# ctu-vras/monoforce

Hardware: AMD Instinct MI355X
Metric: rollout-steps/sec (batch x horizon) on 256x256 terrain (higher is better)
Workload: dtype f32; 1 GPU; c3: B=1024/GPU x T=500 x N=4 contact points, 256x256 grid (res 0.05 m), one shared terrain+friction map (the same on every rank), integrator=odeint-euler (reference default), forward+backward; BASE...; rollouts_per_gpu=1024, rollouts_total=1024, horizon=500, contact_points=4, parallelism=rollout-sharded x1

## Files before the change

monoforce_amd/csrc/rollout_bwd_cp_kernel.h:

```cpp
#pragma once
#include "rollout_bwd_kernel.h"
#include "rollout_cp_common.h"
#include "stream_ring.h"
#include <type_traits>

namespace mf {

#ifdef MF_STREAM_PROFILE
extern __device__ unsigned long long mf_stream_prof[32];
#define MF_PROF_T(v) const unsigned long long v = __builtin_readcyclecounter()
#define MF_PROF_RT(v) const unsigned long long v = __builtin_amdgcn_s_memrealtime()
#define MF_PROF_ACC(name) unsigned long long name = 0
#define MF_PROF_SUM(name, t0) name += __builtin_readcyclecounter() - (t0)
#define MF_PROF_OUT(slot, val) do { if (lane == 0) atomicAdd(&mf_stream_prof[slot], (unsigned long long)(val)); } while (0)
#define MF_PROF_ADD(slot, t0) MF_PROF_OUT(slot, __builtin_readcyclecounter() - (t0))
#define MF_PROF_MAX(slot, val) do { if (lane == 0) atomicMax(&mf_stream_prof[slot], (unsigned long long)(val)); } while (0)
#define MF_PROF_DRAIN() asm volatile("s_waitcnt vmcnt(0) lgkmcnt(0)" ::: "memory")
#else
#define MF_PROF_T(v)
#define MF_PROF_RT(v)
#define MF_PROF_ACC(name)
#define MF_PROF_SUM(name, t0)
#define MF_PROF_OUT(slot, val)
#define MF_PROF_ADD(slot, t0)
// ... 448 lines not shown
      k.wa = mf_fma(wa_s, dpp<kB0>(fr), wa_o); k.wb = mf_fma(wb_s, dpp<kB1>(fr), wb_o);
      k.wq = k.wa * k.wb;
      k.cj = v.q.y; k.wraw = v.q.z; k.A = v.q.w;
      k.idx = v.idx; k.zc = v.zc; k.mcv = has_mu ? v.mc : one;
      k.mub = dot4(k.wq, k.mcv);
      const S dz = v.zc - dpp<kB0>(v.zc);
      const S u = mf_fma(dpp<kN12>(dz), n_mul, n_add);
      k.inl = M::inv_len(dot3(u, u));
      k.nrm = u * k.inl;
      k.inv_csum = M::div(one, sum_points(k.cj));
      k.coln2 = dot3(st.R0, st.R0);
      k.il = M::inv_len(k.coln2);
      k.e = st.R0 * k.il;
      k.tv = cp_track(tv_v, tv_w, st.cv, st.cw);
      k.F0 = -(k.A * k.nrm);
      k.F1 = cp_spring(k.A, k.nrm, k.cj, k.inv_csum);
      k.Fr = M::clamp(k.F1, -mg, mg);
      k.Nn = M::sqrt(dot3(k.Fr, k.Fr));
      k.cmdv = cp_cmd(k.tv, k.e, k.vp);
      k.s = k.mub * k.cmdv;
      k.sn = dot3(k.s, k.nrm);
      k.stv = cp_tangent(k.s, k.sn, k.nrm);
      k.Gf = k.Nn * k.stv;
      const S f = k.Fr + M::clamp(k.Gf, -mg, mg);
      k.f1 = dpp<kRot1>(f); k.f2 = dpp<kRot2>(f);
    };
    const bool loss_on = STREAM && a.loss_gt != nullptr;
    const Msk loss_mask = loss_on ? ~(Msk)0 : (Msk)0;
    const S loss_scale = loss_on ? S(2.0) * a.loss_gloss[0] * a.loss_inv_count : zero;
    const S* const loss_gt_lane = loss_on ? a.loss_gt + ((size_t)b * (size_t)a.loss_T2) * 3u + (unsigned)cc : a.z;
    const int* const l_row_stamp = loss_on ? a.loss_row_stamp : reinterpret_cast<const int*>(a.ts);
    const S* const l_row_w = loss_on ? a.loss_row_w : a.ts;
    const int l_T2m1 = loss_on ? a.loss_T2 - 1 : 0;
    if constexpr (STREAM) {
      const unsigned un = (unsigned)max(n, 0);
      unsigned o3 = v3 + un * s3, o9 = v9 + un * s9, oc = v_ctrl + un * kC, orc = un * rec_step;
      constexpr unsigned kUp = ODE ? 1u : 0u;
      unsigned og_xs = u_xs + (un + kUp) * sg_xs, og_xds = u_xds + (un + kUp) * sg_xds, og_om = u_om + (un + kUp) * sg_om;
      unsigned og_r = u_r + (un + kUp) * sg_r, og_fs = u_fs + (un + kUp) * sg_fs, og_ff = u_ff + (un + kUp) * sg_ff;
      int ti = max(n, 0);
      auto request_state = [&](StateIn& d, Saved& v) {
        d.x = zero;
#ifdef MF_STREAM_NO_FETCH
        d.xd = S(0.1); d.w = S(0.01); d.R0 = cc == 0 ? one : zero; d.R1 = cc == 1 ? one : zero; d.R2 = cc == 2 ? one : zero; d.cv = S(0.5); d.cw = S(0.1);
        d.t1 = S(0.01); d.t0 = zero; v.q = f4v{S(100.3), S(0.2), S(0.1), S(50.0)};
        return;
#endif
        if constexpr (ODE) {
          d.xd = bload1<S>(rXds, o3, 0u); d.w = bload1<S>(rOm, o3, 0u);
          bload3(rRs, o9, 0u, &d.R0, &d.R1, &d.R2);
          d.t1 = a.ts[ti + 1]; d.t0 = a.ts[ti];
        } else {
          const bool init = ti == 0;
          const unsigned p3 = init ? o3 : o3 - s3, p9 = init ? o9 : o9 - s9;
          const S xd = bload1<S>(rXds, p3, 0u), w = bload1<S>(rOm, p3, 0u);
          S R0, R1, R2;
          bload3(rRs, p9, 0u, &R0, &R1, &R2);
          d.xd = init ? ini.xd : xd; d.w = init ? ini.w : w;
          d.R0 = init ? ini.R0 : R0; d.R1 = init ? ini.R1 : R1; d.R2 = init ? ini.R2 : R2;
          d.x = bload1<S>(rOm, o3, 0u);
          d.t1 = a.dt; d.t0 = zero;
        }
        bload2(rCtrl, oc, 0u, &d.cv, &d.cw);
        v.q = __builtin_nontemporal_load(reinterpret_cast<const f4v*>(prec + (size_t)orc));
      };
      auto request_up = [&](UpIn& u) {
#ifdef MF_STREAM_NO_FETCH
        u.gXs = S(0.001);
        if constexpr (!XS_ONLY) { u.gXds = u.gOm = u.gR0 = u.gR1 = u.gR2 = u.gFs = u.gFf = S(0.001); }
        return;
#endif
        u.gXs = bload1<S>(rgXs, og_xs, 0u);
        if constexpr (!XS_ONLY) {
          u.gXds = bload1<S>(rgXds, og_xds, 0u); u.gOm = bload1<S>(rgOm, og_om, 0u);
          bload3(rgRs, og_r, 0u, &u.gR0, &u.gR1, &u.gR2);
          u.gFs = bload1<S>(rgFs, og_fs, 0u); u.gFf = bload1<S>(rgFf, og_ff, 0u);
        }
      };
      auto step_back_up = [&]() {
        og_xs -= sg_xs;
        if constexpr (!XS_ONLY) { og_xds -= sg_xds; og_om -= sg_om; og_r -= sg_r; og_fs -= sg_fs; og_ff -= sg_ff; }
      };
      constexpr int kSlots = SLOTS, kPlanesD = ODE ? 0 : 6, kPlanes = (XS_ONLY ? 10 : 12) + kPlanesD;
      constexpr bool kPow2 = (kSlots & (kSlots - 1)) == 0;
      __shared__ f4v ring[kSlots * kPlanes * 64];
      __shared__ int flags[4];
      typedef __attribute__((address_space(3))) volatile int LdsCounter;
      LdsCounter* vflags = (LdsCounter*)flags;
      if (threadIdx.x == 0) { flags[0] = 0; flags[1] = 0; flags[2] = 0; flags[3] = 0; }
      constexpr unsigned kAnsPlane = 0u, kIdxPlane = 7u * 64u;
      typedef S f2v __attribute__((ext_vector_type(2)));
      if constexpr (HANDOFF) {
        for (unsigned sl = threadIdx.x >> 6; sl < (unsigned)kSlots; sl += 3u) {
          f4v* o = ring + sl * (unsigned)(kPlanes * 64) + lane;
          o[kAnsPlane] = f4v{zero, zero, zero, zero}; o[kIdxPlane] = f4v{zero, zero, zero, idx_as(zero, 0)};
        }
      }
      __syncthreads();
      const bool loss_val = loss_on && a.loss_out != nullptr;
      __shared__ S l_part[3 * 16];
      auto loss_share = [&](S acc) {
        if (!loss_val) return;
        const int wv = (int)(threadIdx.x >> 6);
        if (lane < 16) l_part[wv * 16 + lane] = zero;
        if (p == 0 && q < 3) l_part[wv * 16 + (lane >> 4) * 4 + q] = acc;
        asm volatile("" ::: "memory");
        if (lane == 0) __hip_atomic_fetch_add(&flags[2], 1, __ATOMIC_RELAXED, __HIP_MEMORY_SCOPE_WORKGROUP);
      };
      auto loss_value_finish = [&]() {
        if (!loss_val) return;
        while (__builtin_amdgcn_readfirstlane(vflags[2]) != 3) __builtin_amdgcn_s_sleep(1);
        asm volatile("" ::: "memory");
        unsigned last_wg = 0u;
        if (lane == 0) {
          S tot = zero;
#pragma unroll
          for (int r = 0; r < 4; ++r)
#pragma unroll
            for (int v = 0; v < 3; ++v) tot += (l_part[v * 16 + r * 4 + 0] + l_part[v * 16 + r * 4 + 1]) + l_part[v * 16 + r * 4 + 2];
          __builtin_nontemporal_store(tot, a.loss_partial + blockIdx.x);
          __threadfence();
          last_wg = atomicAdd(a.loss_ticket, 1u) == gridDim.x - 1 ? 1u : 0u;
        }
        last_wg = __builtin_amdgcn_readfirstlane(last_wg);
        if (last_wg) {
          __threadfence();
          const int n_act = min(64, (a.B - (int)blockIdx.x * 4) * 16);
          S tot = zero;
          for (unsigned k0 = (unsigned)lane; k0 < gridDim.x; k0 += 8u * (unsigned)n_act) {
            S v[8];
#pragma unroll
            for (int i = 0; i < 8; ++i) {
              const unsigned k2 = k0 + (unsigned)(i * n_act);
              v[i] = __builtin_nontemporal_load(a.loss_partial + min(k2, gridDim.x - 1u));
              v[i] = k2 < gridDim.x ? v[i] : zero;
            }
#pragma unroll
            for (int i = 0; i < 8; ++i) tot += v[i];
          }
          S sum = zero;
#pragma unroll
          for (int k2 = 0; k2 < 64; ++k2) sum += k2 < n_act ? mf_readlane(tot, k2) : zero;
          if (lane == 0) {
            a.loss_out[0] = sum * a.loss_inv_count;
            *a.loss_ticket = 0u;
          }
        }
      };
      __shared__ S snap_c[4 * 64];
      auto snap_prepare = [&]() {
        if (!a.skip_snap) {
          S wq, dx, dy;
          int idx;
          snap_cell(idx, wq, dx, dy);
          snap_c[lane] = idx_as(zero, idx); snap_c[64 + lane] = wq; snap_c[128 + lane] = dx; snap_c[192 + lane] = dy;
        }
        asm volatile("" ::: "memory");
        vflags[3] = 1;
      };
      if (threadIdx.x >= 64) {
        static_assert(kSlots % BATCH == 0 && (BATCH == 2 || BATCH == 3), "a batch must not wrap around the ring");
        static_assert(!HANDOFF || stream_ring::fixed_ownership(kSlots, BATCH), "hand-off: a wave reads back the answers of the steps it wrote");
        struct Slot { StateIn st; Saved sv; UpIn up; S lg, lw; int sj; };
        unsigned zero_lane = 0u;
        asm("" : "+v"(zero_lane));
        const int fk = __builtin_amdgcn_readfirstlane((int)(threadIdx.x >> 6)) - 1;
        int m = n;
        S l_acc = zero;
        auto fetch = [&](Slot& r) {
          request_state(r.st, r.sv);
          request_up(r.up);
          r.sj = ld32(l_row_stamp, (unsigned)ti + kUp + zero_lane);
          r.lw = ld32(l_row_w, (unsigned)ti + kUp + zero_lane);
          r.lg = zero;
          o3 -= s3; o9 -= s9; oc -= kC; orc -= rec_step; --ti;
          step_back_up();
          --m;
        };
        constexpr unsigned kB = (unsigned)BATCH;
        auto skip3 = [&]() {
          o3 -= kB * s3; o9 -= kB * s9; oc -= kB * kC; orc -= kB * rec_step; ti -= BATCH; m -= BATCH;
          og_xs -= kB * sg_xs;
          if constexpr (!XS_ONLY) { og_xds -= kB * sg_xds; og_om -= kB * sg_om; og_r -= kB * sg_r; og_fs -= kB * sg_fs; og_ff -= kB * sg_ff; }
        };
        MF_PROF_T(t_fetcher);
        MF_PROF_ACC(acc_room); MF_PROF_ACC(acc_pub);
        auto room = [&](int upto) {
          MF_PROF_T(t0);
          while (!stream_ring::has_room(upto - 1, __builtin_amdgcn_readfirstlane(vflags[1]), kSlots)) __builtin_amdgcn_s_sleep(2);
          asm volatile("" ::: "memory");
          MF_PROF_SUM(acc_room, t0);
        };
        int pub = 0;
        auto publish_written = [&](int upto) {
          asm volatile("" ::: "memory");
          if (__builtin_amdgcn_readfirstlane(vflags[0]) == pub) { vflags[0] = upto; pub = upto; }
        };
        auto publish = [&](int upto) {
          asm volatile("" ::: "memory");
          MF_PROF_T(t0);
          if (pub != upto) {
            while (__builtin_amdgcn_readfirstlane(vflags[0]) != pub) __builtin_amdgcn_s_sleep(1);
            asm volatile("" ::: "memory");
            vflags[0] = upto; pub = upto;
          }
          MF_PROF_SUM(acc_pub, t0);
        };
        [[maybe_unused]] auto absorb = [&](unsigned ni, S nz, S nm) {
          const bool same = !act | (ni == acc_idx);
          if (!same) emit(acc_idx, acc_z, acc_m);
          acc_idx = act ? ni : acc_idx;
          acc_z = same ? acc_z + nz : nz;
          acc_m = same ? acc_m + nm : nm;
        };
        [[maybe_unused]] auto absorb_slot = [&](unsigned slot) {
          const f4v* in = ring + slot * (unsigned)(kPlanes * 64) + lane;
          const f2v ans = *reinterpret_cast<const f2v*>(in + kAnsPlane);
          const S ib = reinterpret_cast<const S*>(in + kIdxPlane)[3];
          absorb((unsigned)idx_of(ib), ans.x, ans.y);
        };
        [[maybe_unused]] unsigned pend_idx = 0u;
        [[maybe_unused]] S pend_z = zero, pend_m = zero;
        auto put = [&](const Slot& r, unsigned slot, int o) {
            Rec k;
            rebuild(r.st, r.sv, k);
            if constexpr (HANDOFF) {
              asm("" : "+v"(pend_z), "+v"(pend_m) : "v"(k.zc), "v"(k.mcv), "v"(k.R2), "v"(k.cj), "v"(r.lg), "v"(r.up.gXs));
              absorb(pend_idx, pend_z, pend_m);
            }
            const S mw = inside(k.wraw, -a.omega_max, a.omega_max) ? one : zero;
            const S mG = inside(k.Gf, -mg, mg) ? one : zero;
            const S mF1 = inside(k.F1, -mg, mg) ? one : zero;
            const S invNn = k.Nn > zero ? M::div(one, k.Nn) : zero;
            const S cmask = k.coln2 >= S(1e-12) ? one : zero;
            const S cs = k.cj * k.inv_csum;
            const f4v p0 = f4v{k.R0, k.R1, k.R2, k.h};
            const f4v p1 = f4v{k.w1, k.w2, k.r1, k.r2};
            const f4v p2 = f4v{k.f1, k.f2, mw, mG * k.stv};
            const f4v p3 = f4v{mG * k.Nn, k.nrm, k.s, k.sn};
            const f4v p4 = f4v{k.cmdv, k.mub, k.tv * k.mub, k.Fr * invNn};
            const f4v p5 = f4v{mF1 * cs, mF1 * k.nrm, k.A, -(a.k * cs)};
            const f4v p6 = f4v{-(a.damp * cs), -(k.A * k.inv_csum), k.A * k.cj * k.inv_csum * k.inv_csum, -S(10.0) * k.cj * (one - k.cj)};
            const f4v p7 = f4v{k.vp, -(k.inl * a.inv_res), k.wq, idx_as(zero, k.idx)};
            const f4v p8 = f4v{k.zc, k.mcv, wa_s * k.wb * a.inv_res, wb_s * k.wa * a.inv_res};
            const Msk smask = r.sj >= 0 ? ~(Msk)0 : (Msk)0;
            const S gXs_row = bfi(loss_mask, bfi(smask, cp_loss_grad(loss_scale, r.up.gXs, r.lg, r.lw), zero), r.up.gXs);
            l_acc += bfi(smask, cp_loss_term(r.up.gXs, r.lg, r.lw), zero);
            const f4v p9 = f4v{k.e, k.il, cmask * k.e * k.il, first * gXs_row};
            f4v d0 = {zero, zero, zero, zero}, d1 = d0, d2 = d0, d3 = d0, d4 = d0, d5 = d0;
            if constexpr (!ODE) {
              const S h = a.dt, wn = r.st.x;
              const S th2 = dot3(wn, wn);
              const S idn = M::inv_len(th2);
              const S kv = wn * idn;
              const S th = M::sqrt(th2);
              S sn_, oc;
              M::sincos_small(th * h, &sn_, &oc);
              const S kk = dot3(kv, kv);
              const S kv1 = dpp<kRot1>(kv), kv2 = dpp<kRot2>(kv);
              const S ok = oc * kv;
              const S m0 = mf_fma(ok, kv, mf_fma(-oc, kk, one)), m1 = mf_fma(ok, kv1, -(sn_ * kv2)), m2 = mf_fma(ok, kv2, sn_ * kv1);
              const S q0 = dpp<kB0>(kv), q1 = dpp<kB1>(kv), q2 = dpp<kB2>(kv);
              const S Rk = k.R0 * q0 + k.R1 * q1 + k.R2 * q2;
              const S idn2 = th2 >= S(1e-12) ? idn * idn : zero;
              const S ith = th2 > zero ? M::div(one, th) : zero;
              d0 = f4v{wn, kv, q0, q1};
              d1 = f4v{q2, Rk, kk, sn_};
              d2 = f4v{oc, h * (one - oc), h * sn_, idn};
              d3 = f4v{idn2, ith, dpp<kB0>(m0), dpp<kB0>(m1)};
              d4 = f4v{dpp<kB0>(m2), dpp<kB1>(m2), dpp<kB1>(m0), dpp<kB1>(m1)};
              d5 = f4v{dpp<kB2>(m1), dpp<kB2>(m2), dpp<kB2>(m0), zero};
            }
            room(o + 1);
            f4v* out = ring + slot * (unsigned)(kPlanes * 64) + lane;
            [[maybe_unused]] f2v old_ans = {zero, zero};
            [[maybe_unused]] S old_idx = zero;
            if constexpr (HANDOFF) {
              old_ans = *reinterpret_cast<const f2v*>(out + kAnsPlane);
              old_idx = reinterpret_cast<const S*>(out + kIdxPlane)[3];
              asm volatile("" ::: "memory");
            }
            out[0] = p0; out[64] = p1; out[128] = p2; out[192] = p3; out[256] = p4; out[320] = p5; out[384] = p6; out[448] = p7; out[512] = p8; out[576] = p9;
            if constexpr (!XS_ONLY) {
              out[640] = f4v{first * r.up.gXds, first * r.up.gOm, r.up.gFs, r.up.gFf};
              out[704] = f4v{first * r.up.gR0, first * r.up.gR1, first * r.up.gR2, zero};
            }
            if constexpr (!ODE) {
              constexpr int D0 = (XS_ONLY ? 10 : 12) * 64;
              out[D0] = d0; out[D0 + 64] = d1; out[D0 + 128] = d2; out[D0 + 192] = d3; out[D0 + 256] = d4; out[D0 + 320] = d5;
            }
            publish_written(o + 1);
            if constexpr (HANDOFF) { pend_idx = (unsigned)idx_of(old_idx); pend_z = old_ans.x; pend_m = old_ans.y; }
#ifdef MF_STREAM_PROFILE
            if (o == 0) MF_PROF_ADD(18, t_k0);
#endif
          };
        int ord = BATCH * fk;
        unsigned sbase = kB * (unsigned)fk;
        auto fetch3 = [&](Slot (&s)[BATCH]) {
#pragma unroll
          for (int i = 0; i < BATCH; ++i) fetch(s[i]);
          skip3();
        };
        auto gather1 = [&](Slot& r) {
          gather_cells(r.sv);
          r.lg = loss_gt_lane[(size_t)(unsigned)min(max(r.sj, 0), l_T2m1) * 3u];
        };
        auto gather3 = [&](Slot (&s)[BATCH]) {
#pragma unroll
          for (int i = 0; i < BATCH; ++i) gather1(s[i]);
        };
        auto put3 = [&](const Slot (&s)[BATCH]) {
          pub = ord;
#pragma unroll
          for (int i = 0; i < BATCH; ++i) put(s[i], sbase + (unsigned)i, ord + i);
          publish(ord + BATCH);
          ord += 2 * BATCH;
          if constexpr (kSlots != 2 * BATCH) sbase = sbase + 2u * kB >= (unsigned)kSlots ? sbase + 2u * kB - (unsigned)kSlots : sbase + 2u * kB;
        };
        Slot A[BATCH], B[BATCH], C[BATCH];
        const int n_full = (n + 1) / BATCH;
        int full = (n_full - fk + 1) / 2;
        if (fk == 1) skip3();
        if (full >= 2) {
          fetch3(A); fetch3(B); gather3(A);
          full -= 2;
          while (full >= 3) {
            fetch3(C); gather3(B); put3(A);
            fetch3(A); gather3(C); put3(B);
            fetch3(B); gather3(A); put3(C);
            full -= 3;
          }
          if (full == 0) { gather3(B); put3(A); put3(B); }
          else if (full == 1) { fetch3(C); gather3(B); put3(A); gather3(C); put3(B); put3(C); }
          else { fetch3(C); gather3(B); put3(A); fetch3(A); gather3(C); put3(B); gather3(A); put3(C); put3(A); }
        } else if (full == 1) { fetch3(A); gather3(A); put3(A); }
        if (fk == (n_full & 1)) {
          int o = BATCH * n_full;
          unsigned sl = sbase;
          while (m >= 0) {
            Slot r0;
            fetch(r0);
            gather1(r0);
            pub = o;
            put(r0, sl, o);
            publish(o + 1);
            ++sl; ++o;
          }
        }
        MF_PROF_ADD(2 + 4 * fk, t_fetcher);
        MF_PROF_OUT(0 + 4 * fk, acc_room); MF_PROF_OUT(1 + 4 * fk, acc_pub);
        loss_share(l_acc);
        if (fk == 0) {
          MF_PROF_T(t_lf);
          loss_value_finish();
          MF_PROF_DRAIN();
          MF_PROF_ADD(21, t_lf);
#ifdef MF_STREAM_PROFILE
          MF_PROF_MAX(17, __builtin_readcyclecounter() - t_lf);
          MF_PROF_MAX(14, __builtin_amdgcn_s_memrealtime());
#endif
        } else {
          snap_prepare();
        }
        if constexpr (HANDOFF) {
          MF_PROF_T(t_dr);
          while (__builtin_amdgcn_readfirstlane(vflags[1]) != n_steps) __builtin_amdgcn_s_sleep(1);
          asm volatile("" ::: "memory");
          MF_PROF_ADD(25 + fk, t_dr);
          absorb(pend_idx, pend_z, pend_m);
          for (int o = stream_ring::first_undrained(n_steps, kSlots); o < n_steps; ++o)
            if (stream_ring::owner_of(o, BATCH) == fk) absorb_slot((unsigned)stream_ring::slot_of(o, kSlots));
          if (act) emit(acc_idx, acc_z, acc_m);
        }
        return;
      }
        int consumed = 0, seen = 0;
        unsigned rslot = 0u;
        UpIn uZ;
        load_upstream(0, uZ);
        S l_row0 = zero;
        if (loss_on && ODE) {
          const S g0 = loss_gt_lane[(size_t)max(a.loss_row_stamp[0], 0) * 3u], w0 = a.loss_row_w[0];
          const bool stamped = a.loss_row_stamp[0] >= 0;
          l_row0 = stamped ? cp_loss_term(uZ.gXs, g0, w0) : zero;
          uZ.gXs = stamped ? cp_loss_grad(loss_scale, uZ.gXs, g0, w0) : zero;
        }
        loss_share(l_row0);
        struct Coef {
          S R0, R1, R2, h, w1, w2, r1, r2, f1, f2, mw;
          S stvG, NnG, nrm, s, sn;
          S cmdv, mub, tvm, FrN;
          S csm, nm1, A, kcs;
          S dcs, Aic, Acc, dcj;
          S vp, inlr, wq, zc, mcv, wsb, wsa;
          S e, il, eci;
          int idx;
          unsigned off;
          S wn, kv, q0, q1, q2, Rk, kk, sn_, oc, cga, cgb, idn, idn2, ith;
          S M00, M01, M02, M10, M11, M12, M20, M21, M22;
        };
        MF_PROF_T(t_compute);
        MF_PROF_ACC(acc_wait);
#ifdef MF_STREAM_PROFILE
        unsigned long long acc_wait_early = 0, acc_wait_late = 0, n_waited = 0;
#endif
        auto ensure = [&](int k) {
          MF_PROF_T(t0);
          int have = __builtin_amdgcn_readfirstlane(seen);
          while (have < consumed + k) have = __builtin_amdgcn_readfirstlane(vflags[0]);
          asm volatile("" ::: "memory");
          MF_PROF_SUM(acc_wait, t0);
#ifdef MF_STREAM_PROFILE
          const unsigned long long dt = __builtin_readcyclecounter() - t0;
          if (consumed < 30) acc_wait_early += dt;
          if (consumed >= n_steps - 30) acc_wait_late += dt;
          n_waited += __builtin_amdgcn_readfirstlane(seen) < consumed + k ? 1u : 0u;
#endif
        };
        auto grab = [&](Coef& c, UpIn& up) {
          c.off = (kPow2 ? (unsigned)(consumed & (kSlots - 1)) : rslot) * (unsigned)(kPlanes * 64) + (unsigned)lane;
          const f4v* o = ring + c.off;
          if constexpr (!kPow2) rslot = rslot + 1u == (unsigned)kSlots ? 0u : rslot + 1u;
          const f4v c0 = o[0], c1 = o[64], c2 = o[128], c3 = o[192], c4 = o[256], c5 = o[320], c6 = o[384], c7 = o[448], c8 = o[512], c9 = o[576];
          const S idx_bits = c7.w;
          c.R0 = c0.x; c.R1 = c0.y; c.R2 = c0.z; c.h = c0.w;
          c.w1 = c1.x; c.w2 = c1.y; c.r1 = c1.z; c.r2 = c1.w;
          c.f1 = c2.x; c.f2 = c2.y; c.mw = c2.z; c.stvG = c2.w;
          c.NnG = c3.x; c.nrm = c3.y; c.s = c3.z; c.sn = c3.w;
          c.cmdv = c4.x; c.mub = c4.y; c.tvm = c4.z; c.FrN = c4.w;
          c.csm = c5.x; c.nm1 = c5.y; c.A = c5.z; c.kcs = c5.w;
          c.dcs = c6.x; c.Aic = c6.y; c.Acc = c6.z; c.dcj = c6.w;
          c.vp = c7.x; c.inlr = c7.y; c.wq = c7.z; c.idx = idx_of(idx_bits);
          c.zc = c8.x; c.mcv = c8.y; c.wsb = c8.z; c.wsa = c8.w;
          c.e = c9.x; c.il = c9.y; c.eci = c9.z; up.gXs = c9.w;
          if constexpr (!XS_ONLY) {
            const f4v g0 = o[640];
            const S* g1 = reinterpret_cast<const S*>(o + 704);
            up.gXds = g0.x; up.gOm = g0.y; up.gFs = g0.z; up.gFf = g0.w; up.gR0 = g1[0]; up.gR1 = g1[1]; up.gR2 = g1[2];
          }
          if constexpr (!ODE) {
            constexpr int D0 = (XS_ONLY ? 10 : 12) * 64;
            const f4v e0 = o[D0], e1 = o[D0 + 64], e2 = o[D0 + 128], e3 = o[D0 + 192], e4 = o[D0 + 256];
            const S* e5 = reinterpret_cast<const S*>(o + D0 + 320);
            c.wn = e0.x; c.kv = e0.y; c.q0 = e0.z; c.q1 = e0.w;
            c.q2 = e1.x; c.Rk = e1.y; c.kk = e1.z; c.sn_ = e1.w;
            c.oc = e2.x; c.cga = e2.y; c.cgb = e2.z; c.idn = e2.w;
            c.idn2 = e3.x; c.ith = e3.y; c.M00 = e3.z; c.M01 = e3.w;
            c.M02 = e4.x; c.M10 = e4.y; c.M11 = e4.z; c.M12 = e4.w;
            c.M20 = e5[0]; c.M21 = e5[1]; c.M22 = e5[2];
          }
          ++consumed;
        };
        auto release = [&]() {
          seen = vflags[0];
          asm volatile("" ::: "memory");
          vflags[1] = consumed;
        };
        auto take = [&](Coef& c, UpIn& up) {
          ensure(1); grab(c, up);
          if constexpr (HANDOFF) seen = vflags[0]; else release();
        };
        auto answered = [&](int k) {
          asm volatile("" ::: "memory");
          vflags[1] = k;
        };
        auto chain = [&](int n, const Coef& c, const UpIn& up) {
          const S h = c.h;
          S gFr_up = zero, gFf_up = zero, gxdd, gwd;
          if constexpr (ODE) {
          if constexpr (!XS_ONLY) {
            laFs += act ? up.gFs : zero;
            laFf += act ? up.gFf : zero;
            gFr_up = h * laFs; gFf_up = h * laFf;
          }
          gxdd = h * sum_points(lxd); gwd = h * sum_points(lw);
          lxd = mf_fma(h, lx, lxd);
          const S g0 = h * lR0, g1 = h * lR1, g2 = h * lR2;
          const S g01 = dpp<kRot1>(g0), g02 = dpp<kRot2>(g0), g11 = dpp<kRot1>(g1), g12 = dpp<kRot2>(g1), g21 = dpp<kRot1>(g2), g22 = dpp<kRot2>(g2);
          lw += (dpp<kRot1>(c.R0) * g02 - dpp<kRot2>(c.R0) * g01) + (dpp<kRot1>(c.R1) * g12 - dpp<kRot2>(c.R1) * g11) + (dpp<kRot1>(c.R2) * g22 - dpp<kRot2>(c.R2) * g21);
          lR0 += g01 * c.w2 - g02 * c.w1;
          lR1 += g11 * c.w2 - g12 * c.w1;
          lR2 += g21 * c.w2 - g22 * c.w1;
          } else {
            if constexpr (!XS_ONLY) { gFr_up = act ? up.gFs : zero; gFf_up = act ? up.gFf : zero; }
            const S Lk = lR0 * c.q0 + lR1 * c.q1 + lR2 * c.q2;
            const S Gk0 = dot3(c.R0, Lk), Gk1 = dot3(c.R1, Lk), Gk2 = dot3(c.R2, Lk);
            const S Gt0 = dot3(c.Rk, lR0), Gt1 = dot3(c.Rk, lR1), Gt2 = dot3(c.Rk, lR2);
            const S trG = sum3(c.R0 * lR0 + c.R1 * lR1 + c.R2 * lR2);
            const S a0 = sum3(c.R1 * lR2 - c.R2 * lR1), a1 = sum3(c.R2 * lR0 - c.R0 * lR2), a2 = sum3(c.R0 * lR1 - c.R1 * lR0);
            const S ga = -(c.q0 * a0 + c.q1 * a1 + c.q2 * a2);
            const S gb = (c.q0 * Gk0 + c.q1 * Gk1 + c.q2 * Gk2) - c.kk * trG;
            S gth = ga * c.cga + gb * c.cgb;
            const S ac = mask_or(mask_or(mask_or(zero, a0, lane0), a1, lane1), a2, lane2);
            const S sc = mask_or(mask_or(mask_or(zero, Gk0 + Gt0, lane0), Gk1 + Gt1, lane1), Gk2 + Gt2, lane2);
            const S gk = -(c.sn_ * ac) - c.oc * (S(2.0) * trG * c.kv - sc);
            const S gkw = dot3(gk, c.wn);
            gth = mf_fma(-gkw, c.idn2, gth);
            lw += mf_fma(gth * c.ith, c.wn, gk * c.idn);
            gwd = h * sum_points(lw);
            lxd = mf_fma(h, lx, lxd);
            gxdd = h * sum_points(lxd);
            const S n0 = lR0 * c.M00 + lR1 * c.M01 + lR2 * c.M02;
            const S n1 = lR0 * c.M10 + lR1 * c.M11 + lR2 * c.M12;
            const S n2 = lR0 * c.M20 + lR1 * c.M21 + lR2 * c.M22;
            lR0 = n0; lR1 = n1; lR2 = n2;
          }
          const S mwd = c.mw * gwd;
          const S gtau = J0 * dpp<kB0>(mwd) + J1 * dpp<kB1>(mwd) + J2 * dpp<kB2>(mwd);
          const S gt1 = dpp<kRot1>(gtau), gt2 = dpp<kRot2>(gtau);
          const S gq = mf_fma(gxdd, a.inv_mass, gt1 * c.r2 - gt2 * c.r1);
          S gr = c.f1 * gt2 - c.f2 * gt1;
          S gFr = gFr_up + gq;
          const S gFf_ = gFf_up + gq;
          const S gNn = dot3(gFf_, c.stvG);
          const S gst = c.NnG * gFf_;
          const S gsn = -dot3(gst, c.nrm);
          S gn = gsn * c.s - c.sn * gst;
          const S gslip = mf_fma(gsn, c.nrm, gst);
          const S gmuq = dot3(gslip, c.cmdv);
          const S gcmd = c.mub * gslip;
          S gvp = -gcmd;
          const S ge_p = c.tvm * gslip;
          S gv_p = zero, gwc_p = zero;
          if constexpr (GCTRL) {
            const S gtv = dot3(gcmd, c.e);
            gv_p = tv_v * gtv; gwc_p = tv_w * gtv;
          }
          gFr = mf_fma(gNn, c.FrN, gFr);
          const S gF0 = gFr * c.csm;
          const S d1 = dot3(gFr, c.nm1);
          gn = mf_fma(-c.A, gF0, gn);
          const S gvn = c.dcs * d1;
          gvp = mf_fma(gvn, c.nrm, gvp);
          gn = mf_fma(gvn, c.vp, gn);
          const S gcw = mf_fma(c.Aic, d1, sum_points(c.Acc * d1));
          const S gdh = mf_fma(gcw, c.dcj, c.kcs * d1);
          const S gzq = -gdh;
          const S dotn = dot3(gn, c.nrm);
          const S gg = (gn - dotn * c.nrm) * c.inlr;
          const S ggp = dpp<0x51>(gg);
          const S nz = mf_fma(gzq, c.wq, cgA * gg + cgB * ggp);
          const S nm = gmuq * c.wq;
          if constexpr (HANDOFF) {
            *reinterpret_cast<f2v*>(ring + c.off + kAnsPlane) = f2v{nz, nm};
          } else {
            const unsigned ni = (unsigned)c.idx;
            const bool same = !act | (ni == acc_idx);
            st_pending = !same;
            st_idx = acc_idx; st_z = acc_z; st_m = acc_m;
            acc_idx = act ? ni : acc_idx;
            acc_z = same ? acc_z + nz : nz;
            acc_m = same ? acc_m + nm : nm;
          }
          const S vq = gzq * c.zc + gmuq * c.mcv;
          const S gpx = dot4(vq, c.wsb), gpy = dot4(vq, c.wsa);
          const S gp = mask_or(mask_or(mask_or(zero, gpx, lane0), gpy, lane1), gdh, lane2);
          const S gvp1 = dpp<kRot1>(gvp), gvp2 = dpp<kRot2>(gvp);
          gr += gvp1 * c.w2 - gvp2 * c.w1;
          const S gw_p = c.r1 * gvp2 - c.r2 * gvp1;
          const S qa = gp + gr;
          lx += gp; lxd += gvp; lw += gw_p;
          lR0 = mf_fma(qa, P0, lR0); lR1 = mf_fma(qa, P1, lR1); lR2 = mf_fma(qa, P2, lR2);
          S gv = zero, gwc = zero;
          if constexpr (GCTRL) { gv = sum_points(gv_p); gwc = sum_points(gwc_p); }
          lR0 = mf_fma(-dot3(ge_p, c.e), c.eci, mf_fma(ge_p, c.il, lR0));
          gctrl_pending = __builtin_amdgcn_readfirstlane((unsigned)n * kC); gv_pending = gv; gwc_pending = gwc;
        };
        auto crunch = [&](int n, const Coef& c, const UpIn& up, Coef& c_next, UpIn& up_next, auto more, auto paired) {
          add_upstream_masked(up);
          if constexpr (decltype(paired)::value == 1) grab(c_next, up_next);
          else if constexpr (decltype(paired)::value == 2) {
            grab(c_next, up_next);
            if constexpr (HANDOFF) seen = vflags[0]; else release();
          } else if constexpr (decltype(more)::value) take(c_next, up_next);
          if constexpr (!HANDOFF) flush_stash();
          if constexpr (GCTRL) bstore2(rGctrl, v_ctrl, gctrl_pending, gv_pending, gwc_pending);
#ifdef MF_STREAM_NO_VJP
          asm volatile("" :: "v"(c.R0), "v"(c.w1), "v"(c.f1), "v"(c.NnG), "v"(c.cmdv), "v"(c.csm), "v"(c.dcs), "v"(c.vp), "v"(c.zc), "v"(c.e));
#else
          chain(n, c, up);
#endif
          if constexpr (HANDOFF && decltype(paired)::value != 1) answered(n_steps - n);
        };
        using std::true_type;
        using std::false_type;
        Coef cA, cB;
        if (n_steps > 0) {
          take(cA, uA);
          MF_PROF_ADD(3, t_k0); MF_PROF_OUT(19, acc_wait);
          using single = std::integral_constant<int, 0>;
          for (; n >= 2; n -= 2) {
            ensure(2);
            crunch(n, cA, uA, cB, uB, true_type{}, std::integral_constant<int, 1>{});
            crunch(n - 1, cB, uB, cA, uA, true_type{}, std::integral_constant<int, 2>{});
          }
          if (n == 1) { crunch(1, cA, uA, cB, uB, true_type{}, single{}); crunch(0, cB, uB, cA, uA, false_type{}, single{}); }
          else crunch(0, cA, uA, cB, uB, false_type{}, single{});
        }
        MF_PROF_ADD(9, t_compute);
        MF_PROF_OUT(8, acc_wait);
#ifdef MF_STREAM_PROFILE
        MF_PROF_OUT(22, acc_wait_early); MF_PROF_OUT(23, n_waited); MF_PROF_OUT(24, acc_wait_late);
#endif
        MF_PROF_ADD(20, t_k0);
        MF_PROF_DRAIN();
        MF_PROF_T(t_sw);
        if (!a.skip_snap) {
          while (__builtin_amdgcn_readfirstlane(vflags[3]) == 0) __builtin_amdgcn_s_sleep(1);
          asm volatile("" ::: "memory");
          snap_idx = idx_of(snap_c[lane]); snap_wq = snap_c[64 + lane]; snap_dx = snap_c[128 + lane]; snap_dy = snap_c[192 + lane];
        }
        MF_PROF_DRAIN();
        MF_PROF_ADD(7, t_sw);
        uA = uZ; uB = uZ;
    } else {
      struct Raw { StateIn st; Saved sv; };
      Raw S_[3];
      Rec K_[3];
      UpIn U_[3];
      auto up_row = [&](int m) { return ODE ? max(m + 1, 0) : max(m, 0); };
      auto run = [&](auto rtag, int n) {
        constexpr int R = decltype(rtag)::value, R1 = (R + 1) % 3, R2 = (R + 2) % 3;
        add_upstream_state(U_[R]);
        gather_cells(S_[R1].sv);
#ifndef MF_SAVED_NO_STATE
        load_state(max(n - 3, 0), S_[R].st);
#endif
#ifndef MF_SAVED_NO_REC
        load_saved(max(n - 3, 0), S_[R].sv);
#endif
#ifndef MF_SAVED_NO_UP
        load_upstream(min(up_row(n - 2), a.T - 1), U_[R2]);
#endif
#ifndef MF_SAVED_NO_ATOMIC
        flush_stash();
#endif
        if constexpr (GCTRL) bstore2(rGctrl, v_ctrl, gctrl_pending, gv_pending, gwc_pending);
#ifndef MF_SAVED_NO_VJP
        vjp(n, K_[R], U_[R]);
#endif
#ifndef MF_SAVED_NO_VJP
        asm("" : "+v"(S_[R1].sv.zc), "+v"(S_[R1].sv.mc) : "v"(lR0));
#endif
#ifndef MF_SAVED_NO_REBUILD
        rebuild(S_[R1].st, S_[R1].sv, K_[R1]);
#endif
      };
      const int n0 = max(n, 0);
      load_state(n0, S_[0].st);
      load_saved(n0, S_[0].sv);
      load_upstream(min(up_row(n0), a.T - 1), U_[0]);
      load_state(max(n0 - 1, 0), S_[1].st);
      load_saved(max(n0 - 1, 0), S_[1].sv);
      load_upstream(min(up_row(n0 - 1), a.T - 1), U_[1]);
      load_state(max(n0 - 2, 0), S_[2].st);
      load_saved(max(n0 - 2, 0), S_[2].sv);
      gather_cells(S_[0].sv);
      rebuild(S_[0].st, S_[0].sv, K_[0]);
      __builtin_amdgcn_s_waitcnt(0);
      using std::integral_constant;
      int i = 0;
      for (; i + 2 < n_steps; i += 3) {
        run(integral_constant<int, 0>{}, n0 - i);
        run(integral_constant<int, 1>{}, n0 - i - 1);
        run(integral_constant<int, 2>{}, n0 - i - 2);
      }
      if (i < n_steps) run(integral_constant<int, 0>{}, n0 - i);
      if (i + 1 < n_steps) run(integral_constant<int, 1>{}, n0 - i - 1);
      {
        const int r0 = (n0 + 1) % 3;
        uA = r0 == 0 ? U_[0] : (r0 == 1 ? U_[1] : U_[2]);
        uB = uA;
      }
      n = -1;
    }
  } else {
  load_state(max(n, 0), sA);
// ... 108 lines not shown
```

monoforce_amd/csrc/rollout_cp_common.h:

```cpp
#pragma once
#include "mf_common.h"

namespace mf {
namespace cp {

constexpr int kRot1 = 0x09;
constexpr int kRot2 = 0x52;
constexpr int kB0 = 0x00, kB1 = 0x55, kB2 = 0xAA, kB3 = 0xFF;
constexpr int kXor1 = 0xB1, kXor2 = 0x4E;
constexpr int kN12 = 0xA9;
constexpr int kRor4 = 0x124, kRor8 = 0x128;

template <int CTRL, typename S>
__device__ __forceinline__ S dpp(S v) { return dpp_mov<CTRL>(v); }
template <int CTRL>
__device__ __forceinline__ int dppi(int v) { return __builtin_amdgcn_update_dpp(0, v, CTRL, 0xF, 0xF, true); }

template <typename S> struct MaskOf;
template <> struct MaskOf<float> { typedef unsigned type; };
template <> struct MaskOf<double> { typedef unsigned long long type; };

template <typename S>
__device__ __forceinline__ S sum3(S v) { return (v + dpp<kRot1>(v)) + dpp<kRot2>(v); }
template <typename S>
__device__ __forceinline__ S dot3(S a, S b) {
#pragma clang fp contract(off)
  const S v = a * b;
  return (v + dpp<kRot1>(v)) + dpp<kRot2>(v);
}
__device__ __forceinline__ float mask_or(float acc, float v, unsigned m) {
  return __builtin_bit_cast(float, __builtin_bit_cast(unsigned, acc) | (__builtin_bit_cast(unsigned, v) & m));
}
__device__ __forceinline__ double mask_or(double acc, double v, unsigned long long m) {
  return __builtin_bit_cast(double, __builtin_bit_cast(unsigned long long, acc) | (__builtin_bit_cast(unsigned long long, v) & m));
}
template <typename S>
__device__ __forceinline__ S sum4(S v) { v += dpp<kXor1>(v); return v + dpp<kXor2>(v); }
template <typename S>
__device__ __forceinline__ S dot4(S a, S b) {
#pragma clang fp contract(off)
  S v = a * b;
  v += dpp<kXor1>(v);
  return v + dpp<kXor2>(v);
}
template <typename S>
__device__ __forceinline__ S sum_points(S v) { v += dpp<kRor8>(v); return v + dpp<kRor4>(v); }
template <typename S>
__device__ __forceinline__ S cross_pre(S a, S b) {
#pragma clang fp contract(off)
  return a * dpp<kRot1>(b) - dpp<kRot1>(a) * b;
}
template <typename S>
__device__ __forceinline__ S unrot(S d) { return dpp<kRot1>(d); }

template <typename S>
__device__ __forceinline__ S cp_body_r(S P0, S P1, S P2, S g0, S g1, S g2) {
  return mf_fma(P2, g2, mf_fma(P1, g1, P0 * g0));
}
template <typename S>
__device__ __forceinline__ S cp_vel(S xd, S w, S r) { return xd + unrot(cross_pre(w, r)); }
template <typename S>
__device__ __forceinline__ S cp_track(S tv_v, S tv_w, S cv, S cw) { return mf_fma(tv_v, cv, tv_w * cw); }
template <typename S>
__device__ __forceinline__ S cp_normal_force(S k, S dh, S damp, S vn) { return mf_fma(k, dh, damp * vn); }
template <typename S>
__device__ __forceinline__ S cp_spring(S A, S nrm, S cj, S inv_csum) {
#pragma clang fp contract(off)
  return -(A * nrm) * (cj * inv_csum);
}
template <typename S>
__device__ __forceinline__ S cp_cmd(S tv, S e, S vp) { return mf_fma(tv, e, -vp); }
template <typename S>
__device__ __forceinline__ S cp_tangent(S s, S sn, S nrm) { return mf_fma(-sn, nrm, s); }
template <typename S>
__device__ __forceinline__ S cp_wraw(S I0, S I1, S I2, S Tsum) {
  return mf_fma(I2, dpp<kB2>(Tsum), mf_fma(I1, dpp<kB1>(Tsum), I0 * dpp<kB0>(Tsum)));
}
template <typename S>
__device__ __forceinline__ S cp_loss_term(S xs, S g, S w) {
#pragma clang fp contract(off)
  const S d = xs * w - g * w;
  return d * d;
}
template <typename S>
__device__ __forceinline__ S cp_loss_grad(S scale, S xs, S g, S w) {
#pragma clang fp contract(off)
  return scale * w * (xs * w - g * w);
}
__device__ __forceinline__ float bfi(unsigned m, float a, float b) {
  return __builtin_bit_cast(float, (__builtin_bit_cast(unsigned, a) & m) | (__builtin_bit_cast(unsigned, b) & ~m));
}
__device__ __forceinline__ double bfi(unsigned long long m, double a, double b) {
  return __builtin_bit_cast(double, (__builtin_bit_cast(unsigned long long, a) & m) | (__builtin_bit_cast(unsigned long long, b) & ~m));
}
__device__ __forceinline__ float idx_as(float, int i) { return __builtin_bit_cast(float, i); }
__device__ __forceinline__ double idx_as(double, int i) { return (double)i; }
__device__ __forceinline__ int idx_of(float v) { return __builtin_bit_cast(int, v); }
__device__ __forceinline__ int idx_of(double v) { return (int)v; }
constexpr int kMir2 = 0xA4;

template <typename S>
constexpr unsigned kRecBytesPerLane = 4u * (unsigned)sizeof(S);

using Rsrc = const char*;
__device__ __forceinline__ Rsrc make_rsrc(const void* p) { return reinterpret_cast<const char*>(p); }
template <typename S> struct __attribute__((aligned(sizeof(S)))) Pk2 { S a, b; };
template <typename S> struct __attribute__((aligned(sizeof(S)))) Pk3 { S a, b, c; };
template <typename S>
__device__ __forceinline__ S bload1(Rsrc r, unsigned voff, unsigned soff) { return *reinterpret_cast<const S*>(r + (size_t)soff + (size_t)voff); }
template <typename S>
__device__ __forceinline__ void bload2(Rsrc r, unsigned voff, unsigned soff, S* a, S* b) {
  const Pk2<S> v = *reinterpret_cast<const Pk2<S>*>(r + (size_t)soff + (size_t)voff); *a = v.a; *b = v.b;
}
template <typename S>
__device__ __forceinline__ void bload3(Rsrc r, unsigned voff, unsigned soff, S* a, S* b, S* c) {
  const Pk3<S> v = *reinterpret_cast<const Pk3<S>*>(r + (size_t)soff + (size_t)voff); *a = v.a; *b = v.b; *c = v.c;
}
template <typename S>
__device__ __forceinline__ void bstore1(Rsrc r, unsigned voff, unsigned soff, S a) {
  __builtin_nontemporal_store(a, reinterpret_cast<S*>(const_cast<char*>(r) + (size_t)soff + (size_t)voff));
}
template <typename S>
__device__ __forceinline__ void bstore2(Rsrc r, unsigned voff, unsigned soff, S a, S b) {
  *reinterpret_cast<Pk2<S>*>(const_cast<char*>(r) + (size_t)soff + (size_t)voff) = Pk2<S>{a, b};
}
template <typename S>
__device__ __forceinline__ void bstore3(Rsrc r, unsigned voff, unsigned soff, S a, S b, S c) {
  if constexpr (sizeof(S) == 4) {
    typedef S f3v __attribute__((ext_vector_type(3)));
    typedef f3v __attribute__((aligned(sizeof(S)))) f3u;
    const f3v v = {a, b, c};
    __builtin_nontemporal_store(v, reinterpret_cast<f3u*>(const_cast<char*>(r) + (size_t)soff + (size_t)voff));
  } else {
    S* p = reinterpret_cast<S*>(const_cast<char*>(r) + (size_t)soff + (size_t)voff);
    __builtin_nontemporal_store(a, p); __builtin_nontemporal_store(b, p + 1); __builtin_nontemporal_store(c, p + 2);
  }
// ... 8 lines not shown
```

Measured before the change: 1.506 billion rollout-steps/s.

## Use byte-offset ring addressing and fused DPP FMAs in float backward scan

For float, ring slots are now addressed by running byte offsets with a branchless min-based wrap, so the per-step modulo and multiply address math goes away. The paired grab logic derives the second slot's address from the first. Several cross products and quad-broadcast reductions in the backward chain are rewritten as inline-asm v_fmac_f32_dpp sequences, cutting separate DPP moves and multiplies. The main loop is also reorganized around the consumed count, with an initial s_waitcnt. The hand-written asm and the new offset arithmetic add correctness risk, for example around DPP hazards and wrap edge cases.

```diff
diff --git a/monoforce_amd/csrc/rollout_bwd_cp_kernel.h b/monoforce_amd/csrc/rollout_bwd_cp_kernel.h
--- a/monoforce_amd/csrc/rollout_bwd_cp_kernel.h
+++ b/monoforce_amd/csrc/rollout_bwd_cp_kernel.h
@@ -554,8 +554,11 @@
         if constexpr (!XS_ONLY) { og_xds -= sg_xds; og_om -= sg_om; og_r -= sg_r; og_fs -= sg_fs; og_ff -= sg_ff; }
       };
       constexpr int kSlots = SLOTS, kPlanesD = ODE ? 0 : 6, kPlanes = (XS_ONLY ? 10 : 12) + kPlanesD;
-      constexpr bool kPow2 = (kSlots & (kSlots - 1)) == 0;
       __shared__ f4v ring[kSlots * kPlanes * 64];
+      constexpr bool kRunning = std::is_same<S, float>::value;
+      constexpr unsigned kSlotBytes = (unsigned)(kPlanes * 64 * sizeof(f4v)), kRingBytes = (unsigned)kSlots * kSlotBytes;
+      auto ring_wrap = [](unsigned off) { return min(off, off - kRingBytes); };
+      auto ring_at = [&](unsigned off) { return reinterpret_cast<f4v*>(reinterpret_cast<char*>(ring) + off); };
       __shared__ int flags[4];
       typedef __attribute__((address_space(3))) volatile int LdsCounter;
       LdsCounter* vflags = (LdsCounter*)flags;
@@ -693,7 +696,7 @@
         };
         [[maybe_unused]] unsigned pend_idx = 0u;
         [[maybe_unused]] S pend_z = zero, pend_m = zero;
-        auto put = [&](const Slot& r, unsigned slot, int o) {
+        auto put = [&](const Slot& r, unsigned off, int o) {
             Rec k;
             rebuild(r.st, r.sv, k);
             if constexpr (HANDOFF) {
@@ -744,7 +747,7 @@
               d5 = f4v{dpp<kB2>(m1), dpp<kB2>(m2), dpp<kB2>(m0), zero};
             }
             room(o + 1);
-            f4v* out = ring + slot * (unsigned)(kPlanes * 64) + lane;
+            f4v* out = kRunning ? ring_at(off) : ring + off * (unsigned)(kPlanes * 64) + lane;
             [[maybe_unused]] f2v old_ans = {zero, zero};
             [[maybe_unused]] S old_idx = zero;
             if constexpr (HANDOFF) {
@@ -768,7 +771,8 @@
 #endif
           };
         int ord = BATCH * fk;
-        unsigned sbase = kB * (unsigned)fk;
+        constexpr unsigned kStep = kRunning ? kSlotBytes : 1u;
+        unsigned wbase = kRunning ? kB * (unsigned)fk * kSlotBytes + (unsigned)lane * (unsigned)sizeof(f4v) : kB * (unsigned)fk;
         auto fetch3 = [&](Slot (&s)[BATCH]) {
 #pragma unroll
           for (int i = 0; i < BATCH; ++i) fetch(s[i]);
@@ -785,10 +789,13 @@
         auto put3 = [&](const Slot (&s)[BATCH]) {
           pub = ord;
 #pragma unroll
-          for (int i = 0; i < BATCH; ++i) put(s[i], sbase + (unsigned)i, ord + i);
+          for (int i = 0; i < BATCH; ++i) put(s[i], wbase + (unsigned)i * kStep, ord + i);
           publish(ord + BATCH);
           ord += 2 * BATCH;
-          if constexpr (kSlots != 2 * BATCH) sbase = sbase + 2u * kB >= (unsigned)kSlots ? sbase + 2u * kB - (unsigned)kSlots : sbase + 2u * kB;
+          if constexpr (kSlots != 2 * BATCH) {
+            if constexpr (kRunning) wbase = ring_wrap(wbase + 2u * kB * kSlotBytes);
+            else wbase = wbase + 2u * kB >= (unsigned)kSlots ? wbase + 2u * kB - (unsigned)kSlots : wbase + 2u * kB;
+          }
         };
         Slot A[BATCH], B[BATCH], C[BATCH];
         const int n_full = (n + 1) / BATCH;
@@ -809,7 +816,7 @@
         } else if (full == 1) { fetch3(A); gather3(A); put3(A); }
         if (fk == (n_full & 1)) {
           int o = BATCH * n_full;
-          unsigned sl = sbase;
+          unsigned sl = wbase;
           while (m >= 0) {
             Slot r0;
             fetch(r0);
@@ -817,7 +824,7 @@
             pub = o;
             put(r0, sl, o);
             publish(o + 1);
-            ++sl; ++o;
+            sl += kStep; ++o;
           }
         }
         MF_PROF_ADD(2 + 4 * fk, t_fetcher);
@@ -848,6 +855,7 @@
         return;
       }
         int consumed = 0, seen = 0;
+        unsigned rlast = (unsigned)(kSlots - 1) * kSlotBytes + (unsigned)lane * (unsigned)sizeof(f4v);
         unsigned rslot = 0u;
         UpIn uZ;
         load_upstream(0, uZ);
@@ -890,10 +898,19 @@
           n_waited += __builtin_amdgcn_readfirstlane(seen) < consumed + k ? 1u : 0u;
 #endif
         };
-        auto grab = [&](Coef& c, UpIn& up) {
-          c.off = (kPow2 ? (unsigned)(consumed & (kSlots - 1)) : rslot) * (unsigned)(kPlanes * 64) + (unsigned)lane;
-          const f4v* o = ring + c.off;
-          if constexpr (!kPow2) rslot = rslot + 1u == (unsigned)kSlots ? 0u : rslot + 1u;
+        static_assert(kSlots % 2 == 0, "a trip's first step must not be the ring's last slot plus one");
+        auto grab = [&](Coef& c, UpIn& up, auto ahead, auto first_of_pair) {
+          constexpr unsigned kAhead = (unsigned)decltype(ahead)::value;
+          const f4v* o;
+          if constexpr (!kRunning) {
+            c.off = rslot * (unsigned)(kPlanes * 64) + (unsigned)lane;
+            o = ring + c.off;
+            rslot = rslot + 1u == (unsigned)kSlots ? 0u : rslot + 1u;
+          } else {
+            if constexpr (decltype(first_of_pair)::value) c.off = rlast + kSlotBytes;
+            else { c.off = ring_wrap(rlast + kAhead * kSlotBytes); rlast = c.off; }
+            o = ring_at(c.off);
+          }
           const f4v c0 = o[0], c1 = o[64], c2 = o[128], c3 = o[192], c4 = o[256], c5 = o[320], c6 = o[384], c7 = o[448], c8 = o[512], c9 = o[576];
           const S idx_bits = c7.w;
           c.R0 = c0.x; c.R1 = c0.y; c.R2 = c0.z; c.h = c0.w;
@@ -930,7 +947,7 @@
           vflags[1] = consumed;
         };
         auto take = [&](Coef& c, UpIn& up) {
-          ensure(1); grab(c, up);
+          ensure(1); grab(c, up, std::integral_constant<int, 1>{}, std::false_type{});
           if constexpr (HANDOFF) seen = vflags[0]; else release();
         };
         auto answered = [&](int k) {
@@ -949,11 +966,22 @@
           gxdd = h * sum_points(lxd); gwd = h * sum_points(lw);
           lxd = mf_fma(h, lx, lxd);
           const S g0 = h * lR0, g1 = h * lR1, g2 = h * lR2;
-          const S g01 = dpp<kRot1>(g0), g02 = dpp<kRot2>(g0), g11 = dpp<kRot1>(g1), g12 = dpp<kRot2>(g1), g21 = dpp<kRot1>(g2), g22 = dpp<kRot2>(g2);
-          lw += (dpp<kRot1>(c.R0) * g02 - dpp<kRot2>(c.R0) * g01) + (dpp<kRot1>(c.R1) * g12 - dpp<kRot2>(c.R1) * g11) + (dpp<kRot1>(c.R2) * g22 - dpp<kRot2>(c.R2) * g21);
-          lR0 += g01 * c.w2 - g02 * c.w1;
-          lR1 += g11 * c.w2 - g12 * c.w1;
-          lR2 += g21 * c.w2 - g22 * c.w1;
+          if constexpr (kRunning) {
+            S dw0, dw1, dw2, u0, u1, u2;
+            cp_rot_back(g0, c.R0, c.w1, c.w2, &dw0, &u0);
+            cp_rot_back(g1, c.R1, c.w1, c.w2, &dw1, &u1);
+            cp_rot_back(g2, c.R2, c.w1, c.w2, &dw2, &u2);
+            lw += dpp<kRot1>((dw0 + dw1) + dw2);
+            lR0 += u0;
+            lR1 += u1;
+            lR2 += u2;
+          } else {
+            const S g01 = dpp<kRot1>(g0), g02 = dpp<kRot2>(g0), g11 = dpp<kRot1>(g1), g12 = dpp<kRot2>(g1), g21 = dpp<kRot1>(g2), g22 = dpp<kRot2>(g2);
+            lw += (dpp<kRot1>(c.R0) * g02 - dpp<kRot2>(c.R0) * g01) + (dpp<kRot1>(c.R1) * g12 - dpp<kRot2>(c.R1) * g11) + (dpp<kRot1>(c.R2) * g22 - dpp<kRot2>(c.R2) * g21);
+            lR0 += g01 * c.w2 - g02 * c.w1;
+            lR1 += g11 * c.w2 - g12 * c.w1;
+            lR2 += g21 * c.w2 - g22 * c.w1;
+          }
           } else {
             if constexpr (!XS_ONLY) { gFr_up = act ? up.gFs : zero; gFf_up = act ? up.gFf : zero; }
             const S Lk = lR0 * c.q0 + lR1 * c.q1 + lR2 * c.q2;
@@ -979,10 +1007,17 @@
             lR0 = n0; lR1 = n1; lR2 = n2;
           }
           const S mwd = c.mw * gwd;
-          const S gtau = J0 * dpp<kB0>(mwd) + J1 * dpp<kB1>(mwd) + J2 * dpp<kB2>(mwd);
-          const S gt1 = dpp<kRot1>(gtau), gt2 = dpp<kRot2>(gtau);
-          const S gq = mf_fma(gxdd, a.inv_mass, gt1 * c.r2 - gt2 * c.r1);
-          S gr = c.f1 * gt2 - c.f2 * gt1;
+          S gq, gr;
+          if constexpr (kRunning) {
+            S gtr;
+            cp_cross_pair(cp_colT(J0, J1, J2, mwd), c.r2, c.r1, c.f2, c.f1, &gtr, &gr);
+            gq = mf_fma(gxdd, a.inv_mass, gtr);
+          } else {
+            const S gtau = J0 * dpp<kB0>(mwd) + J1 * dpp<kB1>(mwd) + J2 * dpp<kB2>(mwd);
+            const S gt1 = dpp<kRot1>(gtau), gt2 = dpp<kRot2>(gtau);
+            gq = mf_fma(gxdd, a.inv_mass, gt1 * c.r2 - gt2 * c.r1);
+            gr = c.f1 * gt2 - c.f2 * gt1;
+          }
           S gFr = gFr_up + gq;
           const S gFf_ = gFf_up + gq;
           const S gNn = dot3(gFf_, c.stvG);
@@ -1011,11 +1046,18 @@
           const S gzq = -gdh;
           const S dotn = dot3(gn, c.nrm);
           const S gg = (gn - dotn * c.nrm) * c.inlr;
-          const S ggp = dpp<0x51>(gg);
-          const S nz = mf_fma(gzq, c.wq, cgA * gg + cgB * ggp);
-          const S nm = gmuq * c.wq;
+          S nz, nm;
+          if constexpr (kRunning) {
+            S gcell;
+            cp_cell_terms(cgA, cgB, gg, gmuq, c.wq, &gcell, &nm);
+            nz = mf_fma(gzq, c.wq, gcell);
+          } else {
+            const S ggp = dpp<0x51>(gg);
+            nz = mf_fma(gzq, c.wq, cgA * gg + cgB * ggp);
+            nm = gmuq * c.wq;
+          }
           if constexpr (HANDOFF) {
-            *reinterpret_cast<f2v*>(ring + c.off + kAnsPlane) = f2v{nz, nm};
+            *reinterpret_cast<f2v*>(ring_at(c.off) + kAnsPlane) = f2v{nz, nm};
           } else {
             const unsigned ni = (unsigned)c.idx;
             const bool same = !act | (ni == acc_idx);
@@ -1028,9 +1070,16 @@
           const S vq = gzq * c.zc + gmuq * c.mcv;
           const S gpx = dot4(vq, c.wsb), gpy = dot4(vq, c.wsa);
           const S gp = mask_or(mask_or(mask_or(zero, gpx, lane0), gpy, lane1), gdh, lane2);
-          const S gvp1 = dpp<kRot1>(gvp), gvp2 = dpp<kRot2>(gvp);
-          gr += gvp1 * c.w2 - gvp2 * c.w1;
-          const S gw_p = c.r1 * gvp2 - c.r2 * gvp1;
+          S gw_p;
+          if constexpr (kRunning) {
+            S gvw;
+            cp_cross_pair(gvp, c.w2, c.w1, c.r2, c.r1, &gvw, &gw_p);
+            gr += gvw;
+          } else {
+            const S gvp1 = dpp<kRot1>(gvp), gvp2 = dpp<kRot2>(gvp);
+            gr += gvp1 * c.w2 - gvp2 * c.w1;
+            gw_p = c.r1 * gvp2 - c.r2 * gvp1;
+          }
           const S qa = gp + gr;
           lx += gp; lxd += gvp; lw += gw_p;
           lR0 = mf_fma(qa, P0, lR0); lR1 = mf_fma(qa, P1, lR1); lR2 = mf_fma(qa, P2, lR2);
@@ -1041,9 +1090,9 @@
         };
         auto crunch = [&](int n, const Coef& c, const UpIn& up, Coef& c_next, UpIn& up_next, auto more, auto paired) {
           add_upstream_masked(up);
-          if constexpr (decltype(paired)::value == 1) grab(c_next, up_next);
+          if constexpr (decltype(paired)::value == 1) grab(c_next, up_next, std::integral_constant<int, 1>{}, std::integral_constant<bool, kRunning>{});
           else if constexpr (decltype(paired)::value == 2) {
-            grab(c_next, up_next);
+            grab(c_next, up_next, std::integral_constant<int, kRunning ? 2 : 1>{}, std::false_type{});
             if constexpr (HANDOFF) seen = vflags[0]; else release();
           } else if constexpr (decltype(more)::value) take(c_next, up_next);
           if constexpr (!HANDOFF) flush_stash();
@@ -1053,7 +1102,8 @@
 #else
           chain(n, c, up);
 #endif
-          if constexpr (HANDOFF && decltype(paired)::value != 1) answered(n_steps - n);
+          if constexpr (HANDOFF && kRunning && decltype(paired)::value == 2) answered(consumed - 1);
+          else if constexpr (HANDOFF && decltype(paired)::value != 1) answered(n_steps - n);
         };
         using std::true_type;
         using std::false_type;
@@ -1062,10 +1112,21 @@
           take(cA, uA);
           MF_PROF_ADD(3, t_k0); MF_PROF_OUT(19, acc_wait);
           using single = std::integral_constant<int, 0>;
-          for (; n >= 2; n -= 2) {
-            ensure(2);
-            crunch(n, cA, uA, cB, uB, true_type{}, std::integral_constant<int, 1>{});
-            crunch(n - 1, cB, uB, cA, uA, true_type{}, std::integral_constant<int, 2>{});
+          if constexpr (kRunning) {
+            __builtin_amdgcn_s_waitcnt(0);
+            while (n_steps - consumed >= 2) {
+              const int nn = n_steps - consumed;
+              ensure(2);
+              crunch(nn, cA, uA, cB, uB, true_type{}, std::integral_constant<int, 1>{});
+              crunch(nn - 1, cB, uB, cA, uA, true_type{}, std::integral_constant<int, 2>{});
+            }
+            n = n_steps - consumed;
+          } else {
+            for (; n >= 2; n -= 2) {
+              ensure(2);
+              crunch(n, cA, uA, cB, uB, true_type{}, std::integral_constant<int, 1>{});
+              crunch(n - 1, cB, uB, cA, uA, true_type{}, std::integral_constant<int, 2>{});
+            }
           }
           if (n == 1) { crunch(1, cA, uA, cB, uB, true_type{}, single{}); crunch(0, cB, uB, cA, uA, false_type{}, single{}); }
           else crunch(0, cA, uA, cB, uB, false_type{}, single{});
diff --git a/monoforce_amd/csrc/rollout_cp_common.h b/monoforce_amd/csrc/rollout_cp_common.h
--- a/monoforce_amd/csrc/rollout_cp_common.h
+++ b/monoforce_amd/csrc/rollout_cp_common.h
@@ -52,6 +52,40 @@
 }
 template <typename S>
 __device__ __forceinline__ S unrot(S d) { return dpp<kRot1>(d); }
+
+#define MF_DPP_QP(a, b, c, d) " quad_perm:[" #a "," #b "," #c "," #d "] row_mask:0xf bank_mask:0xf bound_ctrl:1"
+#define MF_DPP_ROT1 MF_DPP_QP(1, 2, 0, 0)
+#define MF_DPP_ROT2 MF_DPP_QP(2, 0, 1, 1)
+__device__ __forceinline__ void cp_rot_back(float g, float R, float w1, float w2, float* d, float* u) {
+  float t = -dpp<kRot1>(R) * g, v = -dpp<kRot2>(g) * w1;
+  asm("v_fmac_f32_dpp %0, %2, %3" MF_DPP_ROT1 "\n\t"
+      "v_fmac_f32_dpp %1, %2, %4" MF_DPP_ROT1
+      : "+v"(t), "+v"(v) : "v"(g), "v"(R), "v"(w2));
+  *d = t; *u = v;
+}
+__device__ __forceinline__ float cp_colT(float J0, float J1, float J2, float m) {
+  float acc = J1 * dpp<kB1>(m);
+  asm("v_fmac_f32_dpp %0, %1, %2" MF_DPP_QP(0, 0, 0, 0) "\n\t"
+      "v_fmac_f32_dpp %0, %1, %3" MF_DPP_QP(2, 2, 2, 2) "\n\t"
+      "s_nop 1"
+      : "+v"(acc) : "v"(m), "v"(J0), "v"(J2));
+  return acc;
+}
+__device__ __forceinline__ void cp_cross_pair(float v, float a1, float a2, float b1, float b2, float* x, float* y) {
+  float p = -dpp<kRot2>(v) * a2, r = -dpp<kRot1>(v) * b1;
+  asm("v_fmac_f32_dpp %0, %2, %3" MF_DPP_ROT1 "\n\t"
+      "v_fmac_f32_dpp %1, %2, %4" MF_DPP_ROT2
+      : "+v"(p), "+v"(r) : "v"(v), "v"(a1), "v"(b2));
+  *x = p; *y = r;
+}
+__device__ __forceinline__ void cp_cell_terms(float cgA, float cgB, float gg, float gmuq, float wq, float* t, float* nm) {
+  float a, b;
+  asm("v_mul_f32 %0, %2, %3\n\t"
+      "v_mul_f32 %1, %5, %6\n\t"
+      "v_fmac_f32_dpp %0, %3, %4" MF_DPP_QP(1, 0, 1, 1)
+      : "=&v"(a), "=&v"(b) : "v"(cgA), "v"(gg), "v"(cgB), "v"(gmuq), "v"(wq));
+  *t = a; *nm = b;
+}
 
 template <typename S>
 __device__ __forceinline__ S cp_body_r(S P0, S P1, S P2, S g0, S g1, S g2) {
```

Result: faster. 1.533 billion rollout-steps/s (median of 6 runs) (+1.8%).
